# lcirrottola/ParMmg

Measured on AMD Instinct MI355X. Metric: new vertices located+interpolated/sec, higher is better.
Workload: dtype f64

## Files before the change

### parmmg_amd/csrc/pmx_bdy.hip

```cpp
#include "pmx_device.h"
#include "pmx_kernels.h"
#include "pmx_internal.h"
#include <algorithm>
#include <cmath>

#define UNSET (-1)

__device__ __constant__ int NXT2d[6] = {1, 2, 0, 1, 2, 0};

template <int CAP> struct RegState {
  int vis[CAP];
  int ovp[CAP], ovf[CAP];
  int nv = 0, no = 0;
  bool over = false;
  __device__ void init(int *, int) {}
  __device__ int &V(int i) { return vis[i]; }
  __device__ int &OP(int i) { return ovp[i]; }
  __device__ int &OF(int i) { return ovf[i]; }
  static constexpr int cap() { return CAP; }
};
struct GlobState {
  int *vis, *ovp, *ovf;
  int nv = 0, no = 0, capv = 0;
  bool over = false;
// ... 603 lines not shown
  for (int64_t k = 1 + (int64_t)blockIdx.x * blockDim.x + threadIdx.x; k <= nt;
       k += (int64_t)gridDim.x * blockDim.x)
    tria_hint_one(tris, xyz, k, grid, g);
}

__device__ int tria_hint(const BdyArgs &A, D3 p) {
  const GridDesc &g = A.g;
  int c[3];
  c[0] = (int)fmin(fmax((p.x - g.lo[0]) * g.inv[0], 0.0), (double)(g.dim[0] - 1));
  c[1] = (int)fmin(fmax((p.y - g.lo[1]) * g.inv[1], 0.0), (double)(g.dim[1] - 1));
  c[2] = (int)fmin(fmax((p.z - g.lo[2]) * g.inv[2], 0.0), (double)(g.dim[2] - 1));
  int k = A.grid[(int64_t)c[0] + (int64_t)g.dim[0] * ((int64_t)c[1] + (int64_t)g.dim[1] * c[2])];
  if (k) return k;
  for (int r = 1; r <= 4; r++)
    for (int dz = -r; dz <= r; dz++)
      for (int dy = -r; dy <= r; dy++)
        for (int dx = -r; dx <= r; dx++) {
          if (max(abs(dx), max(abs(dy), abs(dz))) != r) continue;
          int x = c[0] + dx, y = c[1] + dy, z = c[2] + dz;
          if (x < 0 || y < 0 || z < 0 || x >= g.dim[0] || y >= g.dim[1] || z >= g.dim[2]) continue;
          int kk = A.grid[(int64_t)x + (int64_t)g.dim[0] * ((int64_t)y + (int64_t)g.dim[1] * z)];
          if (kk) return kk;
        }
  return 1;
}

#define BDY_CAP 16
#define OVF_CAP 2048

bool pmx_ctx::size_tria_grid() {
  double ext[3];
  int64_t cells = 1;
  for (int ax = 0; ax < 3; ax++) ext[ax] = std::max(bbhi[ax] - bblo[ax], 1e-300);
  const double area = 2.0 * (ext[0] * ext[1] + ext[1] * ext[2] + ext[0] * ext[2]);
  const double h = std::sqrt(area / std::max(1.0, (double)nt / 8.0));
  for (int ax = 0; ax < 3; ax++) {
    int d = (int)std::ceil(ext[ax] / h * (1.0 - 1e-9));
    d = std::max(1, std::min(d, 1024));
    tgd.dim[ax] = d;
    tgd.lo[ax] = bblo[ax];
    tgd.inv[ax] = (double)d / ext[ax];
    cells *= d;
  }
  tcells = nt > 0 ? cells : 0;
  return !tcells || pmx_call{this, "tria hint grid"}.grow(d_tgrid, (size_t)cells);
}

BdyArgs bdy_args(pmx_ctx *c, const VolArgs &a, bool pointmap) {
  BdyArgs B{};
  B.xyz = c->d_xyz.p; B.tris = c->d_tris.p; B.trn = c->d_trn.p; B.ntrange = c->d_ntrange.p; B.ntlist = c->d_ntlist.p;
  B.sol = c->d_sol.p; B.sd = a.sd; B.q = c->d_qxyz.p; B.kind = c->d_kind.p; B.nq = c->nq; B.nt = c->nt;
  B.hausd = c->hausd; B.grid = c->d_tgrid.p; B.g = c->tgd;
  B.out = c->d_out.p; B.wmask = c->d_wmask.p; B.elem = c->d_elem.p; B.status = c->d_status.p;
  B.steps = c->d_steps.p; B.start = c->d_start.p; B.edge = c->d_edge.p; B.vertex = c->d_vertex.p;
  B.bphi = c->d_bphi.p;
  B.stuck_list = c->d_blist.p; B.stuck_count = c->d_counts.p + 1;
  B.ovf_list = c->d_olist.p; B.ovf_count = c->d_counts.p + 2;
  B.list = c->d_bdylist.p; B.nlist = c->nq_bdy_ub; B.nlist_dev = c->d_nsel.p + 1; B.wstats = c->d_bstat.p;
  if (pointmap) B.grid = a.grid + a.nq;
  return B;
}

void launch_bdy_walks(const BdyArgs &B, int *ows, hipStream_t s, int ovf_threads, bool hashed, bool pointmap) {
  const int64_t nb = (B.nlist + 255) / 256;
  if (pointmap)
    hipLaunchKernelGGL((k_locate_bdy<BDY_CAP, true>), dim3((unsigned)nb), dim3(256), 0, s, B);
  else
    hipLaunchKernelGGL(k_locate_bdy<BDY_CAP>, dim3((unsigned)nb), dim3(256), 0, s, B);
  if (hashed)
    hipLaunchKernelGGL(k_locate_bdy_ovf_hash, dim3(ovf_threads / 64), dim3(64), 0, s, B, ows);
  else
    hipLaunchKernelGGL(k_locate_bdy_ovf, dim3(ovf_threads / 64), dim3(64), 0, s, B, ows, OVF_CAP);
  launch_exh_bdy(B, 256, s);
}

bool pmx_ctx::launch_bdy(const VolArgs &a, hipStream_t s, bool pointmap) {
  const pmx_call C{this, "surface locate", s};
  if (nt < 1) return C.fail("surface points present but the background has no boundary trias");
  if (!C.grow(d_blist, (size_t)nq) || !C.grow(d_olist, (size_t)nq) ||
      !C.grow(d_bphi, (size_t)std::max<int64_t>(nq_bdy_ub, 1)) ||
      (!d_ows.p && !C.grow(d_ows, (size_t)OVF_THREADS * 3 * OVF_CAP)))
    return false;
  if (!pointmap) {
    if (!C.hip(hipMemsetAsync(d_tgrid.p, 0, sizeof(int) * (size_t)tcells, s), "tria hint grid memset")) return false;
    int64_t nb = (nt + 255) / 256;
    if (nb > 4096) nb = 4096;
    hipLaunchKernelGGL(k_tria_hint_build, dim3((unsigned)std::max<int64_t>(nb, 1)), dim3(256), 0, s,
                       d_tris.p, d_xyz.p, nt, d_tgrid.p, tgd);
  }
  launch_bdy_walks(bdy_args(this, a, pointmap), d_ows.p, s, OVF_THREADS, false, pointmap);
  return C.hip(hipGetLastError(), "launch");
}

__global__ __launch_bounds__(64) void k_seq_resolve(BdyArgs A, const int *__restrict__ seq,
                                                    const int *__restrict__ nseq_p, const int *__restrict__ sstart,
                                                    const uint8_t *__restrict__ sw, const int *__restrict__ sbase,
                                                    int *tf, int *pf, int *ctl, int *stk_list,
                                                    unsigned *stk_count, unsigned *nreplay,
                                                    const int *__restrict__ cand, const int *__restrict__ ncand) {
  if (threadIdx.x != 0) return;
  const int nseq = *nseq_p;
  int j = ctl[0];
  int prev = ctl[1];
  if (j >= nseq) return;
  bool dirty = prev < 0;
  if (prev < 0) prev = A.elem[seq[j - 1]];
  const int nc = *ncand;
  int lo = 0, hi = nc;
  while (lo < hi) {
    const int mid = (lo + hi) >> 1;
    if (cand[mid] < j) lo = mid + 1;
    else hi = mid;
  }
  int pos = lo;
  unsigned replays = 0;
  while (j < nseq) {
    if (!dirty) {
      while (pos < nc && cand[pos] < j) pos++;
      if (pos >= nc) break;
      const int c = cand[pos];
      if (c > j) {
        prev = A.elem[seq[c - 1]];
        j = c;
      }
    }
    const int i = seq[j];
    if (!sw[i] && sstart[i] == prev) {
      prev = A.elem[i];
      dirty = false;
      j++;
      continue;
    }
    const D3 p = ld3(A.q, i);
    SeqState st{tf, pf, sbase[i]};
    Bary b;
    int k, edge, vtx, step;
    bool wedged;
    A.start[i] = prev;
    const int r = walk_bdy(A, st, p, prev, sbase[i], k, b, edge, vtx, step, wedged);
    replays++;
    if (r != 1) {
      A.steps[i] = -step;
      stk_list[0] = i;
      *stk_count = 1u;
      ctl[0] = j;
      ctl[2] = 1;
      ctl[3] = i;
      atomicAdd(nreplay, replays);
      return;
    }
    finish_bdy(A, i, k, b, edge, vtx, 1, step);
    prev = k;
    dirty = true;
    j++;
  }
  ctl[0] = nseq;
  ctl[2] = 0;
  atomicAdd(nreplay, replays);
}

void launch_seq_resolve(const BdyArgs &B, const SeqBdyArgs &q, hipStream_t s) {
  hipLaunchKernelGGL(k_seq_resolve, dim3(1), dim3(64), 0, s, B, q.seq, q.nseq, q.sstart, q.sw, q.sbase, q.tf, q.pf,
                     q.ctl, q.stk_list, q.stk_count, q.nreplay, q.cand, q.ncand);
}
void launch_exh_bdy(const BdyArgs &B, int blocks, hipStream_t s) {
  hipLaunchKernelGGL(k_exh_bdy, dim3((unsigned)blocks), dim3(256), 0, s, B);
}
// ... 1 lines not shown
```

### parmmg_amd/csrc/pmx_capi.hip

```cpp
#include <hip/hip_runtime.h>
#include <algorithm>
#include <atomic>
#include <cstdio>
#include <string>
#include <vector>

#include "pmx_transfer.h"
#include "pmx_kernels.h"
#include "pmx_internal.h"

#define PMX_EV_PER_RUN 10

static thread_local std::string noctx_err;

static std::atomic<int> &live_contexts(int device) {
  static std::atomic<int> n[64];
  return n[device & 63];
}
void pmx_set_noctx_error(const char *msg) { noctx_err = msg; }


char *pmx_hstage(pmx_ctx *ctx, size_t bytes) {
  const pmx_call C{ctx};
  if (!C.hip(hipStreamSynchronize(ctx->stream), "pmx_hstage: stream")) return nullptr;
  const size_t cap = std::max<size_t>(bytes + bytes / 4, 1 << 20);
  if (!C.hip(ctx->h_stage.grow(bytes, cap), "hipHostMalloc")) return nullptr;
  return ctx->h_stage.p;
}

bool pmx_ctx::check_device_errors() {
  const pmx_call C{this};
  if (!ran || !d_counts.p) return true;
  unsigned e = 0;
  if (!C.ok(hipMemcpy(&e, d_counts.p + PMX_CNT_ERR, sizeof e, hipMemcpyDeviceToHost),
            "reading the step's device error word failed"))
    return false;
  if (e & PMX_DERR_BARRIER)
    return C.fail("k_fallback: a grid barrier timed out (workgroups not co-resident); the step's "
                  "results are invalid");
  return true;
}

pmx_ctx::~pmx_ctx() {
  pmx_split_free(this);
  pmx_merge_free(this);
  pmx_moveifc_free(this);
}

extern "C" {

pmx_ctx *pmx_create(int device) {
  int n = 0;
  if (hipGetDeviceCount(&n) != hipSuccess || n <= 0) return nullptr;
  if (device < 0) device = 0;
  device %= n;
  if (hipSetDevice(device) != hipSuccess) return nullptr;
  pmx_ctx *ctx = new pmx_ctx();
  ctx->device = device;
  static std::atomic<unsigned> n_created{0};
  const bool odd = (n_created.fetch_add(1) & 1u) != 0;
  auto mk = [](hipStream_t *st) { return hipStreamCreateWithFlags(st, hipStreamNonBlocking) == hipSuccess; };
  bool sok;
  if (!odd)
    sok = mk(&ctx->own) && mk(&ctx->side) && mk(&ctx->up) && mk(&ctx->topo);
  else
    sok = mk(&ctx->topo) && mk(&ctx->up) && mk(&ctx->own) && mk(&ctx->side);
  ctx->stream = ctx->own;
  if (!sok ||
      !ctx->ntets.ev_topo.create(false) || !ctx->ntets.ev.create(false) ||
      ctx->h_nbad.grow(PMX_H_WORDS * sizeof(unsigned), PMX_H_WORDS * sizeof(unsigned)) != hipSuccess ||
      !pmx_create_events(ctx->ev_dl, false) || !pmx_create_events(ctx->ev_eg, false) ||
      !ctx->ev_fork.create(false) || !ctx->ev_fork2.create(false) || !ctx->ev_join.create(false)) {
    pmx_destroy(ctx);
    return nullptr;
  }
  live_contexts(device)++;
  ctx->fallback_share = std::max(2, live_contexts(device).load());
  ctx->fallback_blocks = fallback_coresident_blocks(device, ctx->fallback_share);
  if (ctx->fallback_blocks < 1) {
    pmx_destroy(ctx);
    return nullptr;
  }
  return ctx;
}

void pmx_destroy(pmx_ctx *ctx) {
  if (!ctx) return;
  if (ctx->fallback_share > 0) live_contexts(ctx->device)--;
  if (ctx->peer) pmx_destroy(ctx->peer);
  ctx->peer = nullptr;
  hipSetDevice(ctx->device);
  if (ctx->stream) hipStreamSynchronize(ctx->stream);
  if (ctx->side) hipStreamSynchronize(ctx->side);
  if (ctx->topo) hipStreamSynchronize(ctx->topo);
  if (ctx->up) hipStreamSynchronize(ctx->up);
  if (ctx->side) hipStreamDestroy(ctx->side);
  if (ctx->topo) hipStreamDestroy(ctx->topo);
  if (ctx->up) hipStreamDestroy(ctx->up);
  if (ctx->own) hipStreamDestroy(ctx->own);
  delete ctx;
}

const char *pmx_last_error(pmx_ctx *ctx) {
  if (ctx) return ctx->err.c_str();
  return noctx_err.empty() ? "null context" : noctx_err.c_str();
}

int pmx_set_stream(pmx_ctx *ctx, void *s) {
  if (!ctx) return 0;
  ctx->stream = s ? (hipStream_t)s : ctx->own;
  return 1;
}

int pmx_synchronize(pmx_ctx *ctx) {
  if (!ctx) return 0;
  hipSetDevice(ctx->device);
  PMX_CK(pmx_call{ctx}, hipStreamSynchronize(ctx->stream));
  return ctx->check_device_errors() ? 1 : 0;
}

int pmx_device_info(pmx_ctx *ctx, char *buf, int buflen) {
  if (!ctx) return 0;
  hipDeviceProp_t p;
  PMX_CK(pmx_call{ctx}, hipGetDeviceProperties(&p, ctx->device));
  snprintf(buf, (size_t)buflen, "%s %s CUs=%d HBM=%.1fGB", p.name, p.gcnArchName,
           p.multiProcessorCount, (double)p.totalGlobalMem / 1e9);
  return 1;
}

int64_t pmx_debug_live_allocations(void) { return pmx_live_allocations.load(std::memory_order_relaxed); }


void *pmx_device_alloc(pmx_ctx *ctx, size_t bytes) {
  if (!ctx) return nullptr;
  const pmx_call C{ctx, "pmx_device_alloc"};
  hipSetDevice(ctx->device);
  void *p = nullptr;
  const hipError_t e = hipMalloc(&p, std::max<size_t>(bytes, 1));
  if (!C.ok(e, hipGetErrorString(e))) return nullptr;
  if (!C.ok(hipMemset(p, 0, std::max<size_t>(bytes, 1)), "memset")) {
    hipFree(p);
    return nullptr;
  }
  return p;
}

int pmx_device_free(pmx_ctx *ctx, void *p) {
  if (!ctx) return 0;
  hipSetDevice(ctx->device);
  hipStreamSynchronize(ctx->stream);
  return (p == nullptr || hipFree(p) == hipSuccess) ? 1 : 0;
}

int pmx_device_download(pmx_ctx *ctx, void *host, const void *dev, size_t bytes) {
  if (!ctx) return 0;
  const pmx_call C{ctx};
  if (!host || !dev) return C.fail("pmx_device_download: null pointer");
  hipSetDevice(ctx->device);
  PMX_CK(C, hipMemcpyAsync(host, dev, bytes, hipMemcpyDeviceToHost, ctx->stream));
  PMX_CK(C, hipStreamSynchronize(ctx->stream));
  return 1;
}

int pmx_device_upload(pmx_ctx *ctx, void *dev, const void *host, size_t bytes) {
  if (!ctx) return 0;
  const pmx_call C{ctx};
  if (!host || !dev) return C.fail("pmx_device_upload: null pointer");
  hipSetDevice(ctx->device);
  PMX_CK(C, hipMemcpyAsync(dev, host, bytes, hipMemcpyHostToDevice, ctx->stream));
  PMX_CK(C, hipStreamSynchronize(ctx->stream));
  return 1;
}

}


static void fill_vol_args(pmx_ctx *ctx, const SolDesc &sd, const pmx_run_opts &opts, VolArgs &A) {
  A.xyz = ctx->d_xyz.p; A.tets = ctx->d_tets.p; A.wrec = ctx->d_wrec.p; A.sol = ctx->d_sol.p; A.sd = sd;
  A.q = ctx->d_qxyz.p; A.kind = ctx->d_kind.p; A.nq = ctx->nq; A.ne = ctx->ne;
  A.grid = ctx->d_grid.p; A.g = ctx->grid;
  A.out = ctx->d_out.p; A.wmask = ctx->d_wmask.p;
  A.elem = ctx->d_elem.p; A.status = ctx->d_status.p; A.steps = ctx->d_steps.p;
  A.start = ctx->d_start.p;
  A.stuck_list = ctx->d_list.p; A.stuck_count = ctx->d_counts.p;
  A.tie_list = ctx->d_ties.p; A.tie_count = ctx->d_counts.p + 3;
  A.found = ctx->d_found.p; A.bestk = ctx->d_bestk.p; A.best = ctx->d_best.p;
  A.list = ctx->d_vollist.p; A.nlist = ctx->nq_vol_ub; A.nlist_dev = ctx->d_nsel.p; A.wstats = ctx->d_vstat.p;
  A.max_walk = opts.max_walk > 0 ? opts.max_walk : 512;
  A.const_bit = sd.metric_const ? (1u << sd.imet) : 0u;
  A.inline_ties = (opts.flags & PMX_RUN_NO_INLINE_TIES) ? 0 : 1;
  A.ref_walk = (opts.flags & PMX_RUN_REFERENCE_WALK) ? 1 : 0;
  A.rec_start = (opts.flags & PMX_RUN_RECORD_STARTS) ? 1 : 0;
  A.exp = (opts.flags >> PMX_RUN_EXP_SHIFT) & 0xff;
  if (!ctx->compact_recs ||
      (A.exp != 18 && (uint64_t)ctx->h_nbad.p[PMX_H_FAR] * PMX_WREC_FAR_DIV > (uint64_t)std::max<int64_t>(ctx->ne, 1)))
    A.wrec = nullptr;
  A.far = ctx->h_nbad.p[PMX_H_FAR] > 0 ? 1 : 0;
  if (opts.flags & PMX_RUN_POINTMAP) A.grid = ctx->d_pstart.p;
}

static bool run_flags_valid(int flags, std::string *err) {
  const int pub = PMX_RUN_REFERENCE_WALK | PMX_RUN_NO_INLINE_TIES | PMX_RUN_RECORD_STARTS |
                  PMX_RUN_SERIAL_SURFACE | PMX_RUN_FRESH_BACKGROUND | PMX_RUN_DEBUG_BARRIER_TIMEOUT |
                  PMX_RUN_EAGER_DOWNLOAD | PMX_RUN_SEQUENTIAL_SURFACE | PMX_RUN_SEQUENTIAL_VOLUME |
                  PMX_RUN_POINTMAP;
  if (flags & ~(pub | (0xff << PMX_RUN_EXP_SHIFT))) {
    *err = "pmx_run: unknown flag bits";
    return false;
  }
  const int e = (flags >> PMX_RUN_EXP_SHIFT) & 0xff;
  if (e != 0 && e != 6 && e != 17 && e != 18) {
    *err = "pmx_run: unknown experiment switch";
    return false;
  }
  return true;
}

namespace {
struct Step : pmx_call {
  pmx_run_opts opts{};
  SolDesc sd{};
  int64_t n = 0;
  int S = 0;
  bool pm = false;
  bool fresh = false, derive = false, csr = false;
  bool marks = false;
  bool bdy = false, serial = false;
  bool any_interp = false;
  bool hint_first = false;
  hipStream_t st, side, ss;
  DevEvent *ev = nullptr;
  VolArgs A{};

  Step(pmx_ctx *c, const pmx_run_opts *o) : pmx_call{c, nullptr, c->stream}, st(c->stream), side(c->side), ss(c->side) {
    if (o) opts = *o;
  }
  bool begin();
  bool prefix();
  bool classify_and_hint();
  bool locate();
  bool finish();
  void hint_build();
};

bool Step::begin() {
  ctx->ran = false;
  ctx->eager_nch = 0;
  if (!ctx->have_bg || !ctx->have_pts) return fail("pmx_run: upload background and points first");
  hipSetDevice(ctx->device);
  if (opts.hint_stride < 0 || opts.max_walk < 0) return fail("pmx_run: bad options");
  if (!run_flags_valid(opts.flags, &ctx->err)) return false;
  pm = (opts.flags & PMX_RUN_POINTMAP) != 0;
  if (pm && (opts.flags & (PMX_RUN_SEQUENTIAL_SURFACE | PMX_RUN_SEQUENTIAL_VOLUME)))
    return fail("pmx_run: PMX_RUN_POINTMAP cannot be combined with PMX_RUN_SEQUENTIAL_SURFACE / _VOLUME");
  if (pm && !ctx->have_src)
    return fail("pmx_run: PMX_RUN_POINTMAP needs the sources of the current points (pmx_upload_point_sources)");
  n = ctx->nq;
  if (pm && (!pmx_dgrow(ctx, ctx->d_pstart, (size_t)std::max<int64_t>(2 * n, 1)) ||
             !pmx_dgrow(ctx, ctx->d_pmap, (size_t)(2 * (ctx->np + 1))) || !pmx_dgrow(ctx, ctx->d_pmcnt, 2)))
    return false;
  S = ctx->sd.S;
  if (!pmx_dgrow(ctx, ctx->d_out, (size_t)std::max<int64_t>(n * S, 1))) return false;
  sd = ctx->sd;
  sd.metric_const = (opts.hsiz > 0.0 && sd.imet >= 0) ? 1 : 0;
  for (int s = 0; s < sd.nsol; s++)
    if (!(s == sd.imet && sd.metric_const)) any_interp = true;
  if (opts.timing && !(ev = ctx->next_event_slot())) return false;
  fresh = (opts.flags & PMX_RUN_FRESH_BACKGROUND) != 0;
  derive = !ctx->have_derived || fresh;
  bdy = ctx->nq_bdy_ub > 0;
  csr = bdy && (!ctx->have_csr || fresh);
  serial = (opts.flags & PMX_RUN_SERIAL_SURFACE) != 0;
  ss = serial ? st : side;
  marks = fresh && ctx->ntets.have && n > 0;
  hint_first = marks && any_interp;
  return !marks || ctx->ntets.ensure_tets(st);
}

bool Step::prefix() {
  if (ev) PMX_CK(*this, hipEventRecord(ev[0], st));
  ZeroRanges z{};
  z.add(ctx->d_wmask.p, n);
  z.add(ctx->d_counts.p, 32 * sizeof(unsigned));
  if (!pm) z.add(ctx->d_grid.p, ctx->gcells * (int64_t)sizeof(int));
  launch_prologue(z, st);
  if (bdy && !serial) {
    PMX_CK(*this, hipEventRecord(ctx->ev_fork, st));
    PMX_CK(*this, hipStreamWaitEvent(side, ctx->ev_fork, 0));
  }
  if (ev) PMX_CK(*this, hipEventRecord(ev[3], bdy ? ss : st));
  if (csr) {
    if (!ctx->build_node_trias(ss, fresh)) return false;
    ctx->have_csr = true;
  }
  if (marks && !ctx->ntets.step_marks(st)) return false;
  if (derive) {
    if (bdy && !serial) {
      launch_bg_derive(ctx->d_xyz.p, ctx->np, ctx->grid, ctx->d_xyzq.p, ctx->d_tris.p, 0, ctx->d_trn.p, st);
      launch_bg_derive(ctx->d_xyz.p, 0, ctx->grid, ctx->d_xyzq.p, ctx->d_tris.p, ctx->nt, ctx->d_trn.p, side);
    } else {
      launch_bg_derive(ctx->d_xyz.p, ctx->np, ctx->grid, ctx->d_xyzq.p, ctx->d_tris.p, ctx->nt,
                       ctx->d_trn.p, st);
    }
    ctx->have_derived = true;
  }
  if (fresh && !ctx->rederive(st)) return false;
  if (ev) PMX_CK(*this, hipEventRecord(ev[7], st));
  if (ev) PMX_CK(*this, hipEventRecord(ev[8], st));
  if (pm && (!ctx->have_pmap || fresh)) {
    launch_pmap_build(ctx->d_tets.p, ctx->ne, ctx->d_tris.p, ctx->nt, ctx->np, ctx->d_pmap.p, ctx->d_pmcnt.p, st);
    ctx->have_pmap = true;
  }
  if (ev) PMX_CK(*this, hipEventRecord(ev[9], st));
  return true;
}

void Step::hint_build() {
  if (pm) return;
  const int stride = opts.hint_stride > 0 ? opts.hint_stride : PMX_HINT_STRIDE;
  const bool packed = stride == PMX_HINT_STRIDE;
  launch_hint_build(packed ? ctx->d_tets_s.p : nullptr,
                    packed && ctx->samples_sorted ? ctx->d_tets_sk.p : nullptr, ctx->d_tets.p, ctx->ne,
                    stride, ctx->d_grid.p, ctx->grid, ctx->d_xyzq.p, st,
                    packed && ctx->samples_owner ? ctx->nsamp : -1);
}

bool Step::classify_and_hint() {
  if (hint_first) hint_build();
  if (marks) PMX_CK(*this, hipStreamWaitEvent(st, ctx->ntets.ev, 0));
  if (!ctx->classify(st, marks, pm)) return false;
  if (sd.metric_const)
    launch_const_metric(ctx->d_kind.p, n, ctx->d_out.p, S, sd.off[sd.imet], sd.size[sd.imet],
                        opts.hsiz, ctx->d_wmask.p, sd.imet, st);
  return true;
}

bool Step::locate() {
  if (!any_interp) {
    if (bdy && !serial) {
      PMX_CK(*this, hipEventRecord(ctx->ev_join, side));
      PMX_CK(*this, hipStreamWaitEvent(st, ctx->ev_join, 0));
    }
    if (ev)
      for (int k = 1; k < PMX_EV_PER_RUN; k++)
        if (k != 7 && k != 3 && k != 8 && k != 9) PMX_CK(*this, hipEventRecord(ev[k], st));
    PMX_CK(*this, hipGetLastError());
    return true;
  }
  fill_vol_args(ctx, sd, opts, A);
  if (bdy && !serial) {
    PMX_CK(*this, hipEventRecord(ctx->ev_fork2, st));
    PMX_CK(*this, hipStreamWaitEvent(side, ctx->ev_fork2, 0));
    if (!ctx->launch_bdy(A, side, pm)) return false;
    if (ev) PMX_CK(*this, hipEventRecord(ev[5], side));
    PMX_CK(*this, hipEventRecord(ctx->ev_join, side));
  }
  if (!hint_first) hint_build();
  if (ev) PMX_CK(*this, hipEventRecord(ev[1], st));
  if (ctx->nq_vol_ub) launch_walk(A, st, pm);
  if (ev) PMX_CK(*this, hipEventRecord(ev[2], st));
  if (bdy && !serial) {
    PMX_CK(*this, hipStreamWaitEvent(st, ctx->ev_join, 0));
  } else if (bdy) {
    if (!ctx->launch_bdy(A, st, pm)) return false;
    if (ev) PMX_CK(*this, hipEventRecord(ev[5], st));
  } else if (ev) {
    PMX_CK(*this, hipEventRecord(ev[5], st));
  }
  if (ev) PMX_CK(*this, hipEventRecord(ev[6], st));
  ExhArgs E{};
  E.xyz = ctx->d_xyz.p; E.tets = ctx->d_tets.p; E.ne = ctx->ne; E.q = ctx->d_qxyz.p;
  E.list = ctx->d_list.p; E.count = ctx->d_counts.p; E.found = ctx->d_found.p;
  E.best = ctx->d_best.p; E.bestk = ctx->d_bestk.p;
  E.spin_limit = (opts.flags & PMX_RUN_DEBUG_BARRIER_TIMEOUT) ? 0L : (1L << 26);
  const int share = std::max(2, live_contexts(ctx->device).load());
  if (share != ctx->fallback_share) {
    const int fb = fallback_coresident_blocks(ctx->device, share);
    if (fb < 1) return fail("pmx_run: occupancy query failed");
    ctx->fallback_blocks = fb;
    ctx->fallback_share = share;
  }
  if (ctx->nq_vol_ub) launch_exhaustive(E, A, ctx->fallback_blocks, st);
  ctx->seq_stats_n = -1;
  const bool sq_s = bdy && (opts.flags & PMX_RUN_SEQUENTIAL_SURFACE);
  const bool sq_v = ctx->nq_vol_ub > 0 && (opts.flags & PMX_RUN_SEQUENTIAL_VOLUME);
  if (opts.flags & (PMX_RUN_SEQUENTIAL_SURFACE | PMX_RUN_SEQUENTIAL_VOLUME)) {
    if (!ctx->seq_replay(A, st, sq_s, sq_v)) return false;
    ctx->seq_stats_n = 1;
  }
  if (ev) PMX_CK(*this, hipEventRecord(ev[4], st));
  PMX_CK(*this, hipGetLastError());
  return true;
}

bool Step::finish() {
  ctx->ntets.step_done(marks, sd.metric_const ? (1u << sd.imet) : 0u);
  ctx->out_S = S;
  ctx->out_n = n;
  ctx->located = any_interp;
  if ((opts.flags & PMX_RUN_EAGER_DOWNLOAD) && !ctx->eager_download()) return false;
  if (!ctx->ntets.pack_new_tets()) return false;
  ctx->ran = true;
  return true;
}

}

extern "C" int pmx_run(pmx_ctx *ctx, const pmx_run_opts *o) {
  if (!ctx) return 0;
  Step s(ctx, o);
  return s.begin() && s.prefix() && s.classify_and_hint() && s.locate() && s.finish();
}

bool pmx_ctx::eager_download() {
  const pmx_call C{this};
  eager_nch = 0;
  const int64_t n = nq;
  const int S = sd.S;
  if (n == 0 || S == 0) return true;
  const size_t o_wm = pmx_call::al256((size_t)(n * S) * sizeof(double)), bytes = o_wm + pmx_call::al256((size_t)n);
  if (bytes > h_out.cap) {
    PMX_CK(C, hipStreamSynchronize(stream));
    if (!C.ok(h_out.grow(bytes, bytes + bytes / 4), "pmx_run: pinned staging of the eager download")) return false;
  }
  const int nch = (int)std::max<int64_t>(1, std::min<int64_t>(4, (n * S) >> 21));
  for (int c = 0; c < nch; c++) {
    const int64_t lo = n * c / nch, hi = n * (c + 1) / nch;
    PMX_CK(C, hipMemcpyAsync(h_out.p + (size_t)(lo * S) * sizeof(double), d_out.p + lo * S,
                             (size_t)((hi - lo) * S) * sizeof(double), hipMemcpyDeviceToHost, stream));
    PMX_CK(C, hipMemcpyAsync(h_out.p + o_wm + lo, d_wmask.p + lo, (size_t)(hi - lo), hipMemcpyDeviceToHost, stream));
    PMX_CK(C, hipEventRecord(ev_eg[c], stream));
  }
  eager_nch = nch;
  return true;
}

DevEvent *pmx_ctx::next_event_slot() {
  size_t need = (size_t)(ev_used + 1) * PMX_EV_PER_RUN;
// ... 41 lines not shown
```

### parmmg_amd/csrc/pmx_internal.h

```cpp
#pragma once
#include <hip/hip_runtime.h>
#include <algorithm>
#include <chrono>
#include <cstdio>
#include <cstdlib>
#include <functional>
#include <string>
#include <vector>
#include "pmx_transfer.h"
#include "pmx_kernels.h"
#include "pmx_host.h"
#include "pmx_hostpool.h"

#define PMX_HINT_STRIDE 4
#define PMX_RUN_EXP_SHIFT 16
#define PMX_WREC_FAR_DIV 16

enum {
  PMX_H_NONMANIFOLD_NEXT = 0,
  PMX_H_NONMANIFOLD = 1,
  PMX_H_FAR = 2,
  PMX_H_FAR_NEXT = 3,
  PMX_H_BAD_FANS = 4,
  PMX_H_NSAMP = 5,
  PMX_H_WORDS = 8
};
enum {
  PMX_D_FAR = 0,
  PMX_D_FAR_NEXT = 1,
  PMX_D_FANS_STEP = 2,
  PMX_D_FANS_CHECK = 3,
  PMX_D_NSAMP = 4,
  PMX_D_WORDS = 8
};

struct RecordSet {
  DevBuf<TetRec> *tets;
  DevBuf<WRec> *wrec;
  DevBuf<int4> *sample;
  int d_far, h_nonmanifold, h_far;
};

struct NewTets {
  pmx_ctx *const ctx;
  bool have = false;
  int64_t n = 0;
  bool from_view = false;
  bool pending = false, inflight = false;
  bool marks = false, rows_reset = true;
  bool next_topo = false;
  pmx_points_view view{};
  DevBuf<int4> d_v;
  DevBuf<uint8_t> d_mark;
  PinBuf<char> h;
  DevEvent ev, ev_topo;
  unsigned const_bit = 0;

  explicit NewTets(pmx_ctx *c) : ctx(c) {}
  bool points_begin();
  void view_kept(const pmx_points_view &pv, int64_t ntet);
  bool pack_new_tets();
  bool replace(const int *tetra_v, int64_t tetra_stride, int64_t ne);
  bool step_marks(hipStream_t st);
  void step_done(bool marks_in_step, unsigned step_const_bit);
  bool drain();
  bool drop_next();
  bool take_next(bool wanted);
  void consumed();
  bool ensure_tets(hipStream_t s);
  bool mark_new_tets(int64_t ne, hipStream_t s);
  bool fix_orphans();
  int4 *grow_htets(int64_t ne);
};

struct pmx_ctx {
  int device = 0;
  hipStream_t own = nullptr, stream = nullptr;
  hipStream_t side = nullptr;
  DevEvent ev_fork, ev_fork2, ev_join;
  DevEvent ev_dl[8];
  std::string err;
  int fallback_blocks = 0;
  int fallback_share = 0;
  pmx_ctx *peer = nullptr;
  PinBuf<char> h_stage;

  bool have_bg = false;
  int64_t np = 0, ne = 0, nt = 0;
  double hausd = 0.0;
  SolDesc sd{};
  GridDesc grid{};
  int64_t gcells = 0;
  double bblo[3]{}, bbhi[3]{};
  DevBuf<double> d_xyz;
  DevBuf<TetRec> d_tets;
  DevBuf<WRec> d_wrec;
  DevBuf<unsigned> d_wfar;
  DevBuf<double> d_sol;
  DevBuf<int4> d_tets_s;
  DevBuf<int> d_tets_sk;
  bool samples_sorted = false;
  bool samples_owner = false;
  bool compact_recs = false;
  int sample_mode = 0;
  bool bg_btv = false;
  int64_t nsamp = 0;
  DevBuf<unsigned> d_skey;
  DevBuf<int> d_sidx;
  DevBuf<int4> d_salt;
  DevBuf<char> d_stmp;
  DevBuf<TriRec> d_tris;
  DevBuf<int> d_ntlist, d_ntval;
  DevBuf<unsigned> d_ntkey;
  DevBuf<int2> d_ntrange;
  DevBuf<char> d_nttmp;
  bool have_csr = false;
  bool have_derived = false;
  DevBuf<unsigned long long> d_xyzq;
  DevBuf<Pt4> d_trn;
  DevBuf<int> d_grid;
  bool have_pmap = false;
  DevBuf<unsigned> d_pmap, d_pmcnt;
  bool have_tetv = false;
  DevBuf<int4> d_tetv;

  bool have_pts = false, ran = false;
  int64_t nq = 0;
  int64_t nq_vol_ub = 0, nq_bdy_ub = 0;
  int out_S = -1;
  int64_t out_n = -1;
  bool stepped() const { return ran && have_pts && out_n == nq; }
  DevBuf<int8_t> d_kind;
  DevBuf<uint8_t> d_wmask;
  DevBuf<double> d_out;
  DevBuf<int> d_elem, d_status, d_steps, d_start, d_edge, d_vertex;
  DevBuf<int> d_list, d_found, d_bestk;
  DevBuf<int2> d_ties;
  DevBuf<unsigned long long> d_best;
  DevBuf<unsigned> d_counts;
  DevBuf<int> d_vollist, d_bdylist;
  DevBuf<Pt4> d_bphi;
  bool located = false;
  DevBuf<double> d_msol, d_mout;
  DevBuf<uint8_t> d_mwm;
  std::vector<DevEvent> more_ev;
  int more_ev_used = 0;
  DevBuf<double> d_qxyz;
  DevBuf<int> d_nsel;
  bool have_src = false;
  DevBuf<int> d_qsrc, d_pstart;
  DevBuf<int2> d_ctile;
  DevBuf<uint4> d_vstat, d_bstat;
  DevBuf<int> d_blist, d_olist, d_ows;
  DevBuf<unsigned> d_sqkey;
  DevBuf<int> d_sqidx, d_sqint, d_sqtf, d_sqpf, d_sqtv, d_sqows;
  DevBuf<unsigned long long> d_sqval;
  DevBuf<uint8_t> d_sqw, d_sqflag;
  DevBuf<int> d_sqcand;
  DevBuf<char> d_sqtmp;
  unsigned seq_stats[4] = {0, 0, 0, 0};
  int64_t seq_stats_n = -1;
  DevBuf<int> d_tgrid;
// ... 149 lines not shown
```

### parmmg_amd/csrc/pmx_kernels.h

```cpp
#pragma once
#include "pmx_device.h"

struct GridDesc {
  int dim[3];
  double lo[3];
  double inv[3];
  int qf[3];
};

__host__ __device__ inline int64_t gcell(const GridDesc &g, int x, int y, int z) {
  return (int64_t)x + (int64_t)g.dim[0] * ((int64_t)y + (int64_t)g.dim[1] * z);
}

#define PMX_CNT_ERR 7
#define PMX_DERR_BARRIER 1u

struct VolArgs {
  const double *xyz;
  const TetRec *tets;
  const WRec *wrec;
  const double *sol;
  SolDesc sd;
  const double *q;
  const int8_t *kind;
  int64_t nq, ne;
  const int *grid;
  GridDesc g;
  double *out;
  uint8_t *wmask;
  int *elem, *status, *steps, *start;
  int *stuck_list;
  unsigned *stuck_count;
  int2 *tie_list;
  unsigned *tie_count;
  int *found, *bestk;
  unsigned long long *best;
  const int *list;
  int64_t nlist;
  const int *nlist_dev;
  uint4 *wstats;
  int max_walk;
  unsigned const_bit;
  int inline_ties;
  int ref_walk;
  int rec_start;
  int far;
  int exp;
};

struct BdyArgs {
  const double *xyz;
  const TriRec *tris;
  const Pt4 *trn;
  const int2 *ntrange;
  const int *ntlist;
  const double *sol;
  SolDesc sd;
  const double *q;
  const int8_t *kind;
  int64_t nq, nt;
  double hausd;
  const int *grid;
  GridDesc g;
  double *out;
  uint8_t *wmask;
  int *elem, *status, *steps, *start, *edge, *vertex;
  Pt4 *bphi;
  int *stuck_list;
  unsigned *stuck_count;
  int *ovf_list;
  unsigned *ovf_count;
  const int *list;
  int64_t nlist;
  const int *nlist_dev;
  uint4 *wstats;
  const int *seq_start, *seq_base;
  uint8_t *seq_w;
};

struct ExhArgs {
  const double *xyz;
  const TetRec *tets;
  int64_t ne;
  const double *q;
  const int *list;
  const unsigned *count;
  int *found;
  unsigned long long *best;
  int *bestk;
  long spin_limit;
};

void launch_hint_build(const int4 *packed, const int *kidx, const TetRec *tets, int64_t ne, int stride, int *grid,
                       GridDesc g, const unsigned long long *xyzq, hipStream_t s, int64_t nsamp = -1);
void launch_bg_derive(const double *xyz, int64_t np, GridDesc g, unsigned long long *xyzq,
                      const TriRec *tris, int64_t nt, Pt4 *trn, hipStream_t s);
void launch_walk(const VolArgs &a, hipStream_t s, bool pointmap = false);
void launch_exhaustive(const ExhArgs &e, const VolArgs &v, int blocks, hipStream_t s);
void launch_const_metric(const int8_t *kind, int64_t nq, double *out, int S, int off, int size,
                         double hsiz, uint8_t *wmask, int imet, hipStream_t s);
#define PMX_ZERO_MAX 3
struct ZeroRanges {
  void *p[PMX_ZERO_MAX];
  int64_t bytes[PMX_ZERO_MAX];
  int n;
  void add(void *ptr, int64_t b) {
    if (ptr && b > 0) { p[n] = ptr; bytes[n] = b; n++; }
  }
};
void launch_prologue(const ZeroRanges &z, hipStream_t s);
void launch_tet_conn(const TetRec *src, int64_t n, int4 *dst, hipStream_t s);
void launch_promote(const double *qxyz, const double *out, const uint16_t *qtag, int64_t n, int S, double *xyz,
                    double *sol, uint16_t *ptag, hipStream_t s);
void launch_mark_new_tets(const int4 *tv, int64_t ne, uint8_t *mk, int64_t nmk, hipStream_t s);
struct OrphanRows {
  uint8_t *wmask;
  int *elem, *status, *steps, *start, *edge, *vertex;
  int8_t *kind;
};
void launch_orphans(const uint8_t *mk, int64_t n, uint8_t keep, const OrphanRows &r, hipStream_t s);
void launch_patch_rows(const int4 *ent, const double *vals, int64_t n, int S, double *sol, hipStream_t s);
#define CLS_TILE 16384
inline int64_t cls_tiles(int64_t n) { return (n + CLS_TILE - 1) / CLS_TILE; }
void launch_classify(const uint16_t *tag, const uint8_t *mk, int64_t n, int2 *tcnt, int8_t *kind, int *vlist,
                     int *blist, int *nsel, hipStream_t s);
void launch_pmap_build(const TetRec *tets, int64_t ne, const TriRec *tris, int64_t nt, int64_t np,
                       unsigned *map, unsigned *cnt, hipStream_t s);
struct PointMapArgs {
  const int *src;
  const unsigned *vmap, *tmap;
  int64_t np;
  int *vstart, *bstart;
};
void launch_classify_pointmap(const uint16_t *tag, const uint8_t *mk, int64_t n, int2 *tcnt, int8_t *kind,
                              int *vlist, int *blist, int *nsel, const PointMapArgs &pm, hipStream_t s);

void launch_build_tetrec(const int4 *tv, const int *adja, int64_t ne, int stride, TetRec *tets, int4 *sample,
                         hipStream_t s);
size_t owner_scan_temp_bytes(int64_t np);
bool launch_owner_sample(const TetRec *tets, int64_t ne, int64_t np, unsigned *owner, int *flag, int *pos,
                         int4 *out, int *kidx, unsigned *d_count, unsigned *h_count, void *tmp, size_t tmp_bytes,
                         hipStream_t s);
void launch_build_wrec(const TetRec *tets, int64_t ne, WRec *wr, unsigned *d_nfar, unsigned *h_nfar,
                       hipStream_t s);
struct SeqVolArgs {
  const int *vseq;
  const int *nvseq;
  const int *sstart, *sbase;
  uint8_t *sure;
  int *tf;
  int *ctl;
  int *stk_list;
  unsigned *nreplay;
  const int *cand, *ncand;
};
size_t seqv_ovf_ws_ints();
void launch_seqv_spec(const VolArgs &a, const SeqVolArgs &s, int64_t nmax, int *ws, hipStream_t st);
void launch_seqv_resolve(const VolArgs &a, const SeqVolArgs &s, hipStream_t st);
void launch_seqv_flags(const VolArgs &a, const SeqVolArgs &s, int64_t nmax, uint8_t *flags, hipStream_t st);
#define OVF_THREADS (64 * 64)
#define GHS_SLOTS 4096
#define GHS_WS_INTS (GHS_SLOTS * 6)
void launch_bdy_walks(const BdyArgs &B, int *ows, hipStream_t s, int ovf_threads = OVF_THREADS, bool hashed = false,
                      bool pointmap = false);
void launch_exh_bdy(const BdyArgs &B, int blocks, hipStream_t s);
#define PF_INIT ((int)0x80808080)
struct SeqBdyArgs {
  const int *seq, *nseq;
  const int *sstart, *sbase;
  const uint8_t *sw;
  int *tf, *pf;
  int *ctl;
  int *stk_list;
  unsigned *stk_count;
  unsigned *nreplay;
  const int *cand, *ncand;
};
void launch_seq_resolve(const BdyArgs &B, const SeqBdyArgs &q, hipStream_t s);
int fallback_coresident_blocks(int device, int share);

struct StatArgs {
  const double *xyz;
  int xstride, vbase;
  const TetRec *tets;
// ... 15 lines not shown
```

### parmmg_amd/csrc/pmx_points.hip

```cpp
#include <hip/hip_runtime.h>
#include <algorithm>
#include <atomic>
#include <cmath>
#include <cstring>
#include <string>

#include "pmx_transfer.h"
#include "pmx_kernels.h"
#include "pmx_internal.h"


static inline int4 pack_tet_row(const int *v, int64_t first, int64_t n, bool *bad) {
  if (v[0] <= 0) return make_int4(0, 0, 0, 0);
  int w[4];
  for (int l = 0; l < 4; l++) {
    int64_t j = (int64_t)v[l] - first;
    if (j < 0 || j >= n) { *bad = true; j = 0; }
    w[l] = (int)(j + 1);
  }
  return make_int4(w[0], w[1], w[2], w[3]);
}

static bool pack_tet_rows(const char *tc, int64_t stride, int64_t first, int64_t n, int4 *h, int64_t k0, int64_t k1) {
  bool bad = false;
  par_for(k0, k1, [&](int64_t a, int64_t b) {
    bool bd = false;
    for (int64_t k = a; k < b; k++) {
      const int4 r = pack_tet_row((const int *)(tc + k * stride), first, n, &bd);
      st4(&h[k], r.x, r.y, r.z, r.w);
    }
    if (bd) __atomic_store_n(&bad, true, __ATOMIC_RELAXED);
    std::atomic_thread_fence(std::memory_order_seq_cst);
  });
  return bad;
}

bool NewTets::drain() {
  if (!inflight) return true;
  PMX_CK(pmx_call{ctx}, hipEventSynchronize(ev));
  inflight = false;
  return true;
}

bool NewTets::drop_next() {
  if (!next_topo) return true;
  PMX_CK(pmx_call{ctx}, hipStreamSynchronize(ctx->topo));
  next_topo = false;
  return true;
}

bool NewTets::points_begin() {
  have = false;
  if (!drop_next() || !drain()) return false;
  pending = false;
  marks = false;
  rows_reset = true;
  return true;
}

void NewTets::view_kept(const pmx_points_view &pv, int64_t ntet) {
  view = pv;
  pending = from_view = have = ntet > 0;
  n = ntet;
}

bool NewTets::take_next(bool wanted) {
  const bool prepared = next_topo && wanted;
  next_topo = false;
  return prepared;
}

void NewTets::consumed() { have = false; }

int4 *NewTets::grow_htets(int64_t ne) {
  const size_t bytes = (size_t)(ne + 1) * sizeof(int4);
  if (!pmx_call{ctx}.ok(h.grow(bytes, bytes), "pinned staging of the new tets")) return nullptr;
  return (int4 *)h.p;
}

bool NewTets::mark_new_tets(int64_t ne, hipStream_t s) {
  const pmx_call C{ctx};
  if (ctx->nq < 1) return true;
  PMX_CK(C, hipMemsetAsync(d_mark.p, 0, (size_t)ctx->nq, s));
  launch_mark_new_tets(d_v.p, ne, d_mark.p, ctx->nq, s);
  PMX_CK(C, hipGetLastError());
  return true;
}

bool NewTets::pack_new_tets() {
  const pmx_call C{ctx};
  if (!pending) return true;
  pending = false;
  const pmx_points_view *pv = &view;
  const int64_t nq = ctx->nq, ntet = pv->ne;
  hipStream_t up = ctx->up, topo = ctx->topo;
  Trace tr("new tets");
  int4 *htv = grow_htets(ntet);
  if (!htv) return false;
  const char *tc = (const char *)pv->tetra_v;
  bool bad = false;
  htv[0] = make_int4(0, 0, 0, 0);
  const int64_t nch = std::max<int64_t>(1, std::min<int64_t>(8, ntet >> 20));
  for (int64_t c = 0; c < nch && !bad; c++) {
    const int64_t lo = (c == 0) ? 0 : 1 + ntet * c / nch, hi = 1 + ntet * (c + 1) / nch;
    bad = pack_tet_rows(tc, pv->tetra_stride, pv->first, nq, htv, std::max<int64_t>(lo, 1), hi);
    if (!bad)
      PMX_CK(C, hipMemcpyAsync(d_v.p + lo, htv + lo, (size_t)(hi - lo) * sizeof(int4), hipMemcpyHostToDevice, up));
  }
  if (!bad && nq > 0) {
    if (!mark_new_tets(ntet, up)) return false;
    marks = true;
  }
  PMX_CK(C, hipEventRecord(ev, up));
  inflight = true;
  if (bad) {
    have = false;
    return C.fail("pmx_run: new tet vertex outside [first, last] of the points view");
  }
  tr.mark("pack + dma issued");
  if (ctx->residency && ntet > 0) {
    PMX_CK(C, hipStreamWaitEvent(topo, ev, 0));
    if (!ctx->build_records(d_v.p, nullptr, ntet, nq, ctx->records_next(), topo)) return false;
    PMX_CK(C, hipEventRecord(ev_topo, topo));
    next_topo = true;
  }
  return true;
}

bool NewTets::ensure_tets(hipStream_t s) {
  if (pending && !pack_new_tets()) return false;
  if (inflight) PMX_CK(pmx_call{ctx}, hipStreamWaitEvent(s, ev, 0));
  return true;
}

bool NewTets::step_marks(hipStream_t st) {
  const pmx_call C{ctx};
  PMX_CK(C, hipEventRecord(ctx->ev_fork, st));
  PMX_CK(C, hipStreamWaitEvent(ctx->up, ctx->ev_fork, 0));
  if (!mark_new_tets(n, ctx->up)) return false;
  PMX_CK(C, hipEventRecord(ev, ctx->up));
  inflight = true;
  return true;
}

void NewTets::step_done(bool marks_in_step, unsigned step_const_bit) {
  const_bit = step_const_bit;
  rows_reset = marks_in_step;
  if (marks_in_step) marks = true;
}

bool NewTets::fix_orphans() {
  const pmx_call C{ctx};
  if (rows_reset) return true;
  rows_reset = true;
  if (!ctx->ran || !marks || ctx->nq == 0) return true;
  if (inflight) PMX_CK(C, hipStreamWaitEvent(ctx->stream, ev, 0));
  OrphanRows r{ctx->d_wmask.p, ctx->d_elem.p, ctx->d_status.p, ctx->d_steps.p,
               ctx->d_start.p, ctx->d_edge.p,  ctx->d_vertex.p, ctx->d_kind.p};
  launch_orphans(d_mark.p, ctx->nq, (uint8_t)const_bit, r, ctx->stream);
  PMX_CK(C, hipGetLastError());
  return true;
}

bool NewTets::replace(const int *tetra_v, int64_t tetra_stride, int64_t ne) {
  const pmx_call C{ctx};
  const int64_t first = ctx->pts_first, nq = ctx->nq;
  const char *tc = (const char *)tetra_v;
  if (ctx->ran && from_view) {
    if (!drain()) return false;
    const int4 *old = (const int4 *)h.p;
    bool same = old && !pending && ne == view.ne;
    for (int64_t k = 1; same && k <= ne; k++) {
      bool bad = false;
      const int4 r = pack_tet_row((const int *)(tc + k * tetra_stride), first, nq, &bad);
      if (bad) return C.fail("pmx_upload_new_tets: tet vertex outside the uploaded points");
      const int4 o = old[k];
      same = o.x == r.x && o.y == r.y && o.z == r.z && o.w == r.w;
    }
    if (!same)
      return C.fail("pmx_upload_new_tets: the last step took its orphans from the points view's new tets; "
                    "other tets need another pmx_run");
  }
  have = false;
  if (!drop_next()) return false;
  pending = false;
  if (!drain()) return false;
  int4 *hv = grow_htets(ne);
  if (!hv) return false;
  hv[0] = make_int4(0, 0, 0, 0);
  if (pack_tet_rows(tc, tetra_stride, first, nq, hv, 1, ne + 1))
    return C.fail("pmx_upload_new_tets: tet vertex outside the uploaded points");
  if (!pmx_dgrow(ctx, d_v, (size_t)(ne + 1))) return false;
  PMX_CK(C, hipMemcpyAsync(d_v.p, hv, (size_t)(ne + 1) * sizeof(int4), hipMemcpyHostToDevice, ctx->stream));
  if (from_view && nq > 0) {
    if (!mark_new_tets(ne, ctx->stream)) return false;
    marks = true;
    if (ctx->ran) rows_reset = false;
  }
  PMX_CK(C, hipStreamSynchronize(ctx->stream));
  n = ne;
  have = true;
  return true;
}


extern "C" {

int pmx_upload_points(pmx_ctx *ctx, const pmx_points_view *pv) {
  if (!ctx) return 0;
  const pmx_call C{ctx};
  ctx->have_pts = ctx->ran = false;
  ctx->have_src = false;
  Trace tr("points");
  if (!ctx->ntets.points_begin()) return 0;
  ctx->eager_nch = 0;
  if (!pv) return C.fail("pmx_upload_points: null view");
  (void)hipSetDevice(ctx->device);
  const int64_t n = pv->last - pv->first + 1;
  if (n < 0 || n >= (1LL << 31) || pv->first < 0 || (n > 0 && (!pv->c || pv->stride < 24)))
    return C.fail("pmx_upload_points: bad range or coordinates");
  if (pv->tetra_v && (pv->ne < 0 || pv->tetra_stride < 16)) return C.fail("pmx_upload_points: bad new-tet view");
  const size_t nn = (size_t)std::max<int64_t>(n, 1);
  const int64_t ntet = pv->tetra_v ? pv->ne : 0;
  const size_t o_x = 0, o_tg = o_x + pmx_call::al256(nn * 3 * sizeof(double)),
// ... 140 lines not shown
```

Before: 7.271 billion.

## Run classify on upload stream and fork surface locate earlier; fold memsets into prologue

Adds a new event so classification runs on the upload stream right after marking new tets, which lets the surface-locate fork start as soon as classify finishes instead of after hint building on the main stream. The separate memsets of the mark buffer and the tria hint grid move into the batched zero prologue, which needs a larger zero-range limit. This removes launch and serialization overhead on the main stream, at the cost of more complex cross-stream dependencies. The early path is enabled only when a single context is live on the device.

```diff
diff --git a/parmmg_amd/csrc/pmx_bdy.hip b/parmmg_amd/csrc/pmx_bdy.hip
--- a/parmmg_amd/csrc/pmx_bdy.hip
+++ b/parmmg_amd/csrc/pmx_bdy.hip
@@ -709,7 +709,6 @@
       (!d_ows.p && !C.grow(d_ows, (size_t)OVF_THREADS * 3 * OVF_CAP)))
     return false;
   if (!pointmap) {
-    if (!C.hip(hipMemsetAsync(d_tgrid.p, 0, sizeof(int) * (size_t)tcells, s), "tria hint grid memset")) return false;
     int64_t nb = (nt + 255) / 256;
     if (nb > 4096) nb = 4096;
     hipLaunchKernelGGL(k_tria_hint_build, dim3((unsigned)std::max<int64_t>(nb, 1)), dim3(256), 0, s,
diff --git a/parmmg_amd/csrc/pmx_capi.hip b/parmmg_amd/csrc/pmx_capi.hip
--- a/parmmg_amd/csrc/pmx_capi.hip
+++ b/parmmg_amd/csrc/pmx_capi.hip
@@ -70,7 +70,8 @@
       !ctx->ntets.ev_topo.create(false) || !ctx->ntets.ev.create(false) ||
       ctx->h_nbad.grow(PMX_H_WORDS * sizeof(unsigned), PMX_H_WORDS * sizeof(unsigned)) != hipSuccess ||
       !pmx_create_events(ctx->ev_dl, false) || !pmx_create_events(ctx->ev_eg, false) ||
-      !ctx->ev_fork.create(false) || !ctx->ev_fork2.create(false) || !ctx->ev_join.create(false)) {
+      !ctx->ev_fork.create(false) || !ctx->ev_fork2.create(false) || !ctx->ev_join.create(false) ||
+      !ctx->ev_cls.create(false)) {
     pmx_destroy(ctx);
     return nullptr;
   }
@@ -228,6 +229,8 @@
   bool bdy = false, serial = false;
   bool any_interp = false;
   bool hint_first = false;
+  bool cls_up = false;
+  bool forked = false;
   hipStream_t st, side, ss;
   DevEvent *ev = nullptr;
   VolArgs A{};
@@ -241,13 +244,15 @@
   bool locate();
   bool finish();
   void hint_build();
+  bool fork_surface(hipEvent_t after);
 };
 
 bool Step::begin() {
+  hipSetDevice(ctx->device);
+  if (ctx->ran && (opts.flags & PMX_RUN_FRESH_BACKGROUND) && ctx->ntets.have && !ctx->ntets.fix_orphans()) return false;
   ctx->ran = false;
   ctx->eager_nch = 0;
   if (!ctx->have_bg || !ctx->have_pts) return fail("pmx_run: upload background and points first");
-  hipSetDevice(ctx->device);
   if (opts.hint_stride < 0 || opts.max_walk < 0) return fail("pmx_run: bad options");
   if (!run_flags_valid(opts.flags, &ctx->err)) return false;
   pm = (opts.flags & PMX_RUN_POINTMAP) != 0;
@@ -274,6 +279,7 @@
   ss = serial ? st : side;
   marks = fresh && ctx->ntets.have && n > 0;
   hint_first = marks && any_interp;
+  cls_up = marks && !pm && live_contexts(ctx->device).load() < 2;
   return !marks || ctx->ntets.ensure_tets(st);
 }
 
@@ -283,6 +289,8 @@
   z.add(ctx->d_wmask.p, n);
   z.add(ctx->d_counts.p, 32 * sizeof(unsigned));
   if (!pm) z.add(ctx->d_grid.p, ctx->gcells * (int64_t)sizeof(int));
+  if (marks) z.add(ctx->ntets.d_mark.p, n);
+  if (bdy && any_interp && !pm) z.add(ctx->d_tgrid.p, ctx->tcells * (int64_t)sizeof(int));
   launch_prologue(z, st);
   if (bdy && !serial) {
     PMX_CK(*this, hipEventRecord(ctx->ev_fork, st));
@@ -293,7 +301,7 @@
     if (!ctx->build_node_trias(ss, fresh)) return false;
     ctx->have_csr = true;
   }
-  if (marks && !ctx->ntets.step_marks(st)) return false;
+  if (marks && !ctx->ntets.step_marks(st, cls_up)) return false;
   if (derive) {
     if (bdy && !serial) {
       launch_bg_derive(ctx->d_xyz.p, ctx->np, ctx->grid, ctx->d_xyzq.p, ctx->d_tris.p, 0, ctx->d_trn.p, st);
@@ -325,10 +333,26 @@
                     packed && ctx->samples_owner ? ctx->nsamp : -1);
 }
 
+bool Step::fork_surface(hipEvent_t after) {
+  PMX_CK(*this, hipStreamWaitEvent(side, after, 0));
+  if (!ctx->launch_bdy(A, side, pm)) return false;
+  if (ev) PMX_CK(*this, hipEventRecord(ev[5], side));
+  PMX_CK(*this, hipEventRecord(ctx->ev_join, side));
+  forked = true;
+  return true;
+}
+
 bool Step::classify_and_hint() {
-  if (hint_first) hint_build();
-  if (marks) PMX_CK(*this, hipStreamWaitEvent(st, ctx->ntets.ev, 0));
-  if (!ctx->classify(st, marks, pm)) return false;
+  if (any_interp) fill_vol_args(ctx, sd, opts, A);
+  if (cls_up) {
+    if (any_interp && bdy && !serial && !sd.metric_const && !fork_surface(ctx->ev_cls)) return false;
+    if (hint_first) hint_build();
+    PMX_CK(*this, hipStreamWaitEvent(st, ctx->ev_cls, 0));
+  } else {
+    if (hint_first) hint_build();
+    if (marks) PMX_CK(*this, hipStreamWaitEvent(st, ctx->ntets.ev, 0));
+    if (!ctx->classify(st, marks, pm)) return false;
+  }
   if (sd.metric_const)
     launch_const_metric(ctx->d_kind.p, n, ctx->d_out.p, S, sd.off[sd.imet], sd.size[sd.imet],
                         opts.hsiz, ctx->d_wmask.p, sd.imet, st);
@@ -347,13 +371,9 @@
     PMX_CK(*this, hipGetLastError());
     return true;
   }
-  fill_vol_args(ctx, sd, opts, A);
-  if (bdy && !serial) {
+  if (bdy && !serial && !forked) {
     PMX_CK(*this, hipEventRecord(ctx->ev_fork2, st));
-    PMX_CK(*this, hipStreamWaitEvent(side, ctx->ev_fork2, 0));
-    if (!ctx->launch_bdy(A, side, pm)) return false;
-    if (ev) PMX_CK(*this, hipEventRecord(ev[5], side));
-    PMX_CK(*this, hipEventRecord(ctx->ev_join, side));
+    if (!fork_surface(ctx->ev_fork2)) return false;
   }
   if (!hint_first) hint_build();
   if (ev) PMX_CK(*this, hipEventRecord(ev[1], st));
diff --git a/parmmg_amd/csrc/pmx_internal.h b/parmmg_amd/csrc/pmx_internal.h
--- a/parmmg_amd/csrc/pmx_internal.h
+++ b/parmmg_amd/csrc/pmx_internal.h
@@ -61,14 +61,14 @@
   void view_kept(const pmx_points_view &pv, int64_t ntet);
   bool pack_new_tets();
   bool replace(const int *tetra_v, int64_t tetra_stride, int64_t ne);
-  bool step_marks(hipStream_t st);
+  bool step_marks(hipStream_t st, bool cls);
   void step_done(bool marks_in_step, unsigned step_const_bit);
   bool drain();
   bool drop_next();
   bool take_next(bool wanted);
   void consumed();
   bool ensure_tets(hipStream_t s);
-  bool mark_new_tets(int64_t ne, hipStream_t s);
+  bool mark_new_tets(int64_t ne, hipStream_t s, bool zeroed = false);
   bool fix_orphans();
   int4 *grow_htets(int64_t ne);
 };
@@ -77,7 +77,7 @@
   int device = 0;
   hipStream_t own = nullptr, stream = nullptr;
   hipStream_t side = nullptr;
-  DevEvent ev_fork, ev_fork2, ev_join;
+  DevEvent ev_fork, ev_fork2, ev_join, ev_cls;
   DevEvent ev_dl[8];
   std::string err;
   int fallback_blocks = 0;
diff --git a/parmmg_amd/csrc/pmx_kernels.h b/parmmg_amd/csrc/pmx_kernels.h
--- a/parmmg_amd/csrc/pmx_kernels.h
+++ b/parmmg_amd/csrc/pmx_kernels.h
@@ -99,7 +99,7 @@
 void launch_exhaustive(const ExhArgs &e, const VolArgs &v, int blocks, hipStream_t s);
 void launch_const_metric(const int8_t *kind, int64_t nq, double *out, int S, int off, int size,
                          double hsiz, uint8_t *wmask, int imet, hipStream_t s);
-#define PMX_ZERO_MAX 3
+#define PMX_ZERO_MAX 5
 struct ZeroRanges {
   void *p[PMX_ZERO_MAX];
   int64_t bytes[PMX_ZERO_MAX];
diff --git a/parmmg_amd/csrc/pmx_points.hip b/parmmg_amd/csrc/pmx_points.hip
--- a/parmmg_amd/csrc/pmx_points.hip
+++ b/parmmg_amd/csrc/pmx_points.hip
@@ -78,10 +78,10 @@
   return (int4 *)h.p;
 }
 
-bool NewTets::mark_new_tets(int64_t ne, hipStream_t s) {
+bool NewTets::mark_new_tets(int64_t ne, hipStream_t s, bool zeroed) {
   const pmx_call C{ctx};
   if (ctx->nq < 1) return true;
-  PMX_CK(C, hipMemsetAsync(d_mark.p, 0, (size_t)ctx->nq, s));
+  if (!zeroed) PMX_CK(C, hipMemsetAsync(d_mark.p, 0, (size_t)ctx->nq, s));
   launch_mark_new_tets(d_v.p, ne, d_mark.p, ctx->nq, s);
   PMX_CK(C, hipGetLastError());
   return true;
@@ -133,13 +133,17 @@
   return true;
 }
 
-bool NewTets::step_marks(hipStream_t st) {
+bool NewTets::step_marks(hipStream_t st, bool cls) {
   const pmx_call C{ctx};
   PMX_CK(C, hipEventRecord(ctx->ev_fork, st));
   PMX_CK(C, hipStreamWaitEvent(ctx->up, ctx->ev_fork, 0));
-  if (!mark_new_tets(n, ctx->up)) return false;
+  if (!mark_new_tets(n, ctx->up, true)) return false;
   PMX_CK(C, hipEventRecord(ev, ctx->up));
   inflight = true;
+  if (cls) {
+    if (!ctx->classify(ctx->up, true, false)) return false;
+    PMX_CK(C, hipEventRecord(ctx->ev_cls, ctx->up));
+  }
   return true;
 }
 
```

New measurement: 7.356 billion, median of 6. 1.2% higher.
